# fan-ziqi/robot_lab

Hardware: AMD Instinct MI355X
Metric: env-steps/sec (whole node) at 4096 envs/GPU, A1 Velocity-Rough (higher is better)
Workload: dtype f32; 1 GPU; RobotLab-Isaac-Velocity-Rough-Unitree-A1-v0, 4096 envs/GPU, random actions U(-1,1), seed 42+rank; envs_per_gpu=4096, parallelism=env-shard x1, step_kernel=specialised (spec_id 1), envs_per_wavefront=4

## Files before the change

robot_lab_amd/csrc/env_spec.h:

```cpp
#pragma once
#include <string.h>

#include "env_tables.h"

namespace rl {

struct RewSpec {
  int kind;
  float weight;
  float p[4];
  uint32_t joint_mask;
  uint64_t body_mask;
  int n_idx;
  int idx_a[16], idx_b[16];
};
struct ObsSpec {
  int kind;
  float scale, clip_lo, clip_hi, noise_lo, noise_hi;
  int has_noise, offset;
};
struct NoSpec {
  static constexpr bool ON = false;
  static constexpr int ID = 0;
  static constexpr uint32_t SLOT_VALID = ~0u;
// ... 15 lines not shown
    if (kd == 37  || kd == 38 )
      for (int i = 0; i < SP::REW[t].n_idx; ++i) m |= 1ull << SP::REW[t].idx_a[i];
  }
  return m;
}
template <class SP>
constexpr int spec_axis_kind(int j) {
  if constexpr (SP::ON) return SP::AXIS_KIND[j];
  else return 3;
}
template <class LT>
inline int table_axis_kind(const LT& L, int j) {
  int kind = 3;
  for (int i = 0; i < 3; ++i) {
    const float a = L.axis[j][i], b = L.axis[j][(i + 1) % 3], c = L.axis[j][(i + 2) % 3];
    if ((a == 1.0f || a == -1.0f) && b == 0.0f && c == 0.0f) kind = i;
  }
  return kind;
}
template <class SP>
constexpr uint32_t spec_slot_valid() {
#ifdef RL_SLOT_VALID_ALL
  return ~0u;
#else
  return SP::SLOT_VALID;
#endif
}
template <class SP>
constexpr bool spec_slot_any(int s, int spl, int g_lo, int g_hi) {
  for (int g = g_lo; g <= g_hi; ++g)
    if ((spec_slot_valid<SP>() >> (g * spl + s)) & 1u) return true;
  return false;
}
constexpr bool spec_kind_supported(int kd) {
  return kd >= 0 && kd <= 38;
}

template <class SP>
inline bool spec_matches(const TablesT<TopoMax>& T) {
  auto same = [](float a, float b) { return memcmp(&a, &b, 4) == 0; };
  if (T.CL != SP::TP::CL || T.NW != SP::TP::NW || (T.merged != 0) != (SP::TP::M0 != 0) || (T.rotpad != 0) != (SP::TP::NW == 0 && SP::TP::PAD) || T.D != SP::D ||
      T.n_bodies != SP::N_BODIES)
    return false;
  if (T.n_rewards != SP::N_REW || T.cur_lin || T.cur_ang) return false;
  if (T.slot_valid != SP::SLOT_VALID) return false;
  for (int j = 0; j < SP::TP::CL; ++j)
    for (int k = 0; k < NLANE; ++k)
      if (SP::AXIS_KIND[j] != 3 && table_axis_kind(T.lane[k], j) != SP::AXIS_KIND[j]) return false;
  int owned = 0;
  for (int k = 0; k < NLANE; ++k)
    for (int j = 0; j < T.CL + T.NW; ++j) {
      const int jid = T.lane[k].joint_own[j] ? T.lane[k].joint_id[j] : -1;
      if (jid < 0) continue;
      ++owned;
      if (jid >= SP::D || SP::JOINT_K[jid] != k || SP::JOINT_J[jid] != j) return false;
    }
  if (owned != SP::D) return false;
  for (int t = 0; t < SP::N_REW; ++t) {
    const RewTab& R = T.rew[t];
    const RewSpec& Q = SP::REW[t];
    if (R.kind != Q.kind || !same(R.weight, Q.weight) || R.joint_mask != Q.joint_mask || R.body_mask != Q.body_mask || R.n_idx != Q.n_idx) return false;
    for (int i = 0; i < 4; ++i)
      if (!same(R.p[i], Q.p[i])) return false;
    const int nidx = R.kind == 20  ? 4 : R.n_idx;
    for (int i = 0; i < nidx; ++i)
      if (T.idx_pool_a[R.idx_off + i] != Q.idx_a[i] || T.idx_pool_b[R.idx_off + i] != Q.idx_b[i]) return false;
// ... 19 lines not shown
```

robot_lab_amd/csrc/env_step.h:

```cpp
#pragma once
#include <type_traits>

#include "env_spec.h"
#include "env_tables.h"

#if !defined(RL_NO_PK) && !defined(RL_PK)
#define RL_PK 1
#endif
#if defined(RL_PHASE_MARKS) && defined(__HIP_DEVICE_COMPILE__)
#define RL_PHASE(id, name) asm volatile("; PHASE " name)
#elif defined(RL_PHASE_CLOCK) && defined(__HIP_DEVICE_COMPILE__)
#define RL_PHASE(id, name) this->phase_stamp(id)
#define RL_PHASE_START() (this->ph_t0 = 0, this->ph_cur = 0)
#define RL_PHASE_CLOCK_ON 1
#else
#define RL_PHASE(id, name) ((void)0)
#endif
#ifndef RL_PHASE_START
#define RL_PHASE_START() ((void)0)
#endif
constexpr int RL_PHASE_ROW0 = 24;
constexpr int RL_PHASE_SLOTS = 32;

namespace rl {

template <int N>
struct SymIdx {
  static constexpr int size = N * (N + 1) / 2;
  static constexpr int at(int i, int j) { return i <= j ? i * N - i * (i - 1) / 2 + (j - i) : j * N - j * (j - 1) / 2 + (i - j); }
};

template <int I, int N, class F>
RL_FN void static_for(F&& f) {
  if constexpr (I < N) {
    f(std::integral_constant<int, I>{});
    static_for<I + 1, N>(f);
  }
}
template <int I, class F>
RL_FN void static_for_down(F&& f) {
  if constexpr (I >= 0) {
    f(std::integral_constant<int, I>{});
    static_for_down<I - 1>(f);
  }
}

RL_FN float comp(V3 v, int i) { return i == 0 ? v.x : i == 1 ? v.y : v.z; }
RL_FN V3 unit(int i) { return {i == 0 ? 1.f : 0.f, i == 1 ? 1.f : 0.f, i == 2 ? 1.f : 0.f}; }
RL_FN V3 ld3(const float* p) { return {p[0], p[1], p[2]}; }

struct Uni {
  float dt, inv_dt, gravity, contact_k, contact_c, inv_phi_ref, contact_ct, contact_vdep, contact_vstick, limit_k, limit_c, force_threshold;
  float inv_hscale, x0, y0;
  int is_plane, nx, ny;
  double x0d, y0d, inv_hd;
// ... 641 lines not shown
    k = ctx.k();
    sub = ctx.sub();
    li = k * SUB + sub;
    Np = S.Npad;
#pragma unroll
    for (int i = 0; i < MAXOWN; ++i) {
      if constexpr (SUB == 8) own[i] = -1;
      else own[i] = SUB == 1 ? i : (SUB == 2 ? L.own_slot2[sub & 1][i < LaneTabT<TP>::MAXOWN2 ? i : 0] : L.own_slot[sub & 3][i < LaneTabT<TP>::MAXOWN ? i : 0]);
    }
    if constexpr (SUB == 8) {
      int n = 0;
#pragma unroll
      for (int sl = 0; sl < NBS; ++sl) {
        const bool mine = (L.slot_body[sl] >= 0 || (sl == 0 && L.base_body_local >= 0)) && (L.slot_grp[sl] & 7) == sub;
#pragma unroll
        for (int i = 0; i < MAXOWN; ++i) own[i] = (mine && n == i) ? sl : own[i];
        n += mine ? 1 : 0;
      }
    }
    tim.set_own(own); hist_n.set_own(own); cf.set_own(own); fric.set_own(own);
    if constexpr (STATE_BUF) {
      lt_b = Ctx::state_buf(ctx.uniform_ptr(S.lane_state + (size_t)ctx.tile() * ((size_t)LY.NF_LANE * ROW)), (uint32_t)LY.NF_LANE * ROW * (uint32_t)sizeof(float));
      et_b = Ctx::state_buf(ctx.uniform_ptr(S.env_state + (size_t)ctx.tile() * ((size_t)LY.NF_ENV * EPT)), (uint32_t)LY.NF_ENV * (uint32_t)EPT * (uint32_t)sizeof(float));
      lt_off = (uint32_t)sizeof(float) * (uint32_t)(ctx.env_in_tile() * NLANE + k);
      et_off = (uint32_t)sizeof(float) * (uint32_t)ctx.env_in_tile();
    } else {
      lt = S.lane_state + (size_t)ctx.tile() * ((size_t)LY.NF_LANE * ROW) + (uint32_t)(ctx.env_in_tile() * NLANE + k);
      et = S.env_state + (size_t)ctx.tile() * ((size_t)LY.NF_ENV * EPT) + (uint32_t)ctx.env_in_tile();
    }
  }
#ifdef RL_PHASE_CLOCK_ON
  long long ph_t0 = 0;
  int ph_cur = 0;
  __device__ __forceinline__ void phase_stamp(int id) {
    __builtin_amdgcn_s_waitcnt(0);
    const long long t = (long long)__builtin_readcyclecounter();
    if (ctx.lane == 0 && ph_t0 != 0) {
      float* row = S.rew_terms + (size_t)RL_PHASE_ROW0 * (size_t)S.Npad + (size_t)ctx.tile() * RL_PHASE_SLOTS;
      row[ph_cur] += (float)(t - ph_t0);
    }
    ph_cur = id;
    __builtin_amdgcn_s_waitcnt(0);
    ph_t0 = (long long)__builtin_readcyclecounter();
  }
#endif
  RL_FN auto LF(int f) const {
    if constexpr (STATE_BUF) {
      const uint32_t o = (uint32_t)f * ROW * (uint32_t)sizeof(float);
      return __builtin_constant_p(f) ? BufRef{lt_b, lt_off, o} : BufRef{lt_b, lt_off + o, 0u};
    } else return PtrRef{lt + (uint32_t)f * ROW};
  }
  RL_FN auto EF(int f) const {
    if constexpr (STATE_BUF) {
      const uint32_t o = (uint32_t)f * (uint32_t)EPT * (uint32_t)sizeof(float);
      return __builtin_constant_p(f) ? BufRef{et_b, et_off, o} : BufRef{et_b, et_off + o, 0u};
    } else return PtrRef{et + (uint32_t)f * (uint32_t)EPT};
  }
  static constexpr bool M0 = TP::M0 != 0;
  static constexpr int G0 = M0 ? 1 : 0;
  RL_FN int grp_of(int it) const { return G0 + sub + SUB * it; }
  static constexpr bool slot_live(int it, int s) {
    const int lo = G0 + SUB * it, hi = lo + SUB - 1 < CL ? lo + SUB - 1 : CL;
    return spec_slot_any<SP>(s, SPL, lo, hi);
  }
  RL_FN bool owns_group(int g) const { return SUB == 1 || (g < G0 ? sub == 0 : ((g - G0) % SUB) == sub); }
  RL_FN bool on_base(int g, int s) const { return M0 && ((L.sph_base_mask >> (g * SPL + s)) & 1u) != 0u; }
  RL_FN static SV pick_sv(bool c, const SV& a, const SV& b) {
    return SV{{c ? a.a.x : b.a.x, c ? a.a.y : b.a.y, c ? a.a.z : b.a.z}, {c ? a.l.x : b.l.x, c ? a.l.y : b.l.y, c ? a.l.z : b.l.z}};
  }
  RL_FN uint32_t base_bits() const { return M0 ? L.sph_base_mask : ((1u << SPL) - 1u); }
  RL_FN bool owns_slot(int s) const { return owns_group(L.slot_grp[s]); }

  RL_FN void load() {
    pos = {EF(LY.EF_ROOT + 0), EF(LY.EF_ROOT + 1), EF(LY.EF_ROOT + 2)};
    quat = {EF(LY.EF_ROOT + 3), EF(LY.EF_ROOT + 4), EF(LY.EF_ROOT + 5), EF(LY.EF_ROOT + 6)};
    vlin = {EF(LY.EF_ROOT + 7), EF(LY.EF_ROOT + 8), EF(LY.EF_ROOT + 9)};
    vang = {EF(LY.EF_ROOT + 10), EF(LY.EF_ROOT + 11), EF(LY.EF_ROOT + 12)};
    extF = {EF(LY.EF_WRENCH + 0), EF(LY.EF_WRENCH + 1), EF(LY.EF_WRENCH + 2)};
    extT = {EF(LY.EF_WRENCH + 3), EF(LY.EF_WRENCH + 4), EF(LY.EF_WRENCH + 5)};
    base_com = {EF(LY.EF_BASE_COM + 0), EF(LY.EF_BASE_COM + 1), EF(LY.EF_BASE_COM + 2)};
    if (NW > 0) wr_com = {EF(LY.EF_WR_COM + 0), EF(LY.EF_WR_COM + 1), EF(LY.EF_WR_COM + 2)};
    else wr_com = base_com;
#pragma unroll
    for (int j = 0; j < CL; ++j) {
      q[j] = LF(LY.LF_Q + j);
      qd[j] = LF(LY.LF_QD + j);
      kp[j] = LF(LY.LF_KP + j);
      kd[j] = LF(LY.LF_KD + j);
      act[j] = LF(LY.LF_ACT + j);
    }
#pragma unroll
    for (int i = 0; i < NW; ++i) {
      q[CL + i] = EF(LY.EF_TQ + i);
      qd[CL + i] = EF(LY.EF_TQD + i);
      kp[CL + i] = EF(LY.EF_TKP + i);
      kd[CL + i] = EF(LY.EF_TKD + i);
      act[CL + i] = EF(LY.EF_TACT + i);
    }
#pragma unroll
    for (int j = 0; j < JX; ++j) {
      tau_app[j] = 0.f;
      qacc[j] = 0.f;
    }
    if (M0) {
#pragma unroll
// ... 1505 lines not shown
```

robot_lab_amd/csrc/env_terms.h:

```cpp
#pragma once
#include "env_spec.h"
#include "env_step.h"

namespace rl {

enum RewKind {
  REW_TRACK_LIN_VEL_XY_EXP = 0, REW_TRACK_ANG_VEL_Z_EXP, REW_LIN_VEL_Z_L2, REW_ANG_VEL_XY_L2, REW_JOINT_TORQUES_L2,
  REW_JOINT_ACC_L2, REW_JOINT_POS_LIMITS, REW_JOINT_POWER, REW_STAND_STILL, REW_JOINT_POS_PENALTY, REW_JOINT_MIRROR,
  REW_ACTION_RATE_L2, REW_UNDESIRED_CONTACTS, REW_CONTACT_FORCES, REW_FEET_CONTACT_WITHOUT_CMD, REW_FEET_HEIGHT_BODY,
  REW_UPWARD, REW_FEET_AIR_TIME, REW_FEET_AIR_TIME_VARIANCE, REW_FEET_SLIDE, REW_FEET_GAIT, REW_FLAT_ORIENTATION_L2,
  REW_IS_TERMINATED, REW_JOINT_DEVIATION_L1, REW_JOINT_VEL_L2, REW_FEET_CONTACT, REW_FEET_STUMBLE, REW_FEET_HEIGHT,
  REW_TRACK_LIN_VEL_XY_YAW_FRAME_EXP, REW_TRACK_ANG_VEL_Z_WORLD_EXP, REW_FEET_AIR_TIME_POSITIVE_BIPED,
  REW_HANDSTAND_FEET_HEIGHT_EXP, REW_HANDSTAND_FEET_ON_AIR, REW_HANDSTAND_FEET_AIR_TIME, REW_HANDSTAND_ORIENTATION_L2, REW_BASE_HEIGHT_L2, REW_WHEEL_VEL_PENALTY,
  REW_FEET_DISTANCE_Y_EXP, REW_FEET_DISTANCE_XY_EXP, REW_ACTION_MIRROR, REW_ACTION_SYNC
};
enum ObsKind {
  OBS_BASE_LIN_VEL = 0, OBS_BASE_ANG_VEL, OBS_PROJECTED_GRAVITY, OBS_VELOCITY_COMMANDS, OBS_JOINT_POS_REL,
  OBS_JOINT_VEL_REL, OBS_LAST_ACTION, OBS_HEIGHT_SCAN, OBS_JOINT_POS_REL_NO_WHEEL
};

enum { JS_TAU2 = 0, JS_ACC2, JS_QD2, JS_LIMIT, JS_POWER, JS_DEV1, JS_DEV2, JS_DA2, JS_Q, JS_ABSQD, JS_ROWS };
enum { BT_HMAX = 0, BT_CA, BT_CC, BT_LA, BT_LC, BT_FX, BT_FY, BT_FZ, BT_PX, BT_PY, BT_PZ, BT_VX, BT_VY, BT_VZ, BT_NF };
static_assert(JS_ROWS == REW_JS_ROWS && BT_NF == REW_BT_NF && BT_FX == REW_BT_NS, "reward tables: LDS sizing in env_tables.h");

// ... 309 lines not shown
  using Base::pos; using Base::quat; using Base::vlin; using Base::vang; using Base::q; using Base::qd; using Base::kp; using Base::kd;
  using Base::act; using Base::prev_act; using Base::tim; using Base::cf; using Base::hist_n; using Base::tau_app; using Base::qacc;
  using Base::extF; using Base::extT; using Base::base_com; using Base::wr_com;

  V3 cmd;
  float heading_target, cmd_time_left, metric_xy, metric_yaw, push_left;
  static constexpr bool DEFER_LOG = SUB > 1;
  static constexpr int NACC_M = (MAX_T + LPE - 1) / LPE;
  float log_sum[NACC_M], log_mxy, log_myaw;
  bool is_heading, is_standing;
  int level, ttype;
  V3 origin;
  long long ep_len;
  M3 Rwb;
  V3 lin_b, ang_b, grav_b, lin_w;
  float yaw_c, yaw_s;

  RL_FN EnvProgram(Ctx& c, const KState& s) : Base(c, s) {}

  RL_FN void load_task() {
    cmd = {this->EF(LY.EF_CMD + CMD_VX), this->EF(LY.EF_CMD + CMD_VY), this->EF(LY.EF_CMD + CMD_WZ)};
    heading_target = this->EF(LY.EF_CMD + CMD_HEADING);
    cmd_time_left = this->EF(LY.EF_CMD + CMD_TIME_LEFT);
    metric_xy = this->EF(LY.EF_CMD + CMD_METRIC_XY);
    metric_yaw = this->EF(LY.EF_CMD + CMD_METRIC_YAW);
    push_left = this->EF(LY.EF_CMD + CMD_PUSH_LEFT);
    int f = S.flags[e];
    is_heading = f & 1;
    is_standing = (f >> 1) & 1;
    level = S.level[e];
    ttype = S.ttype[e];
    origin = {this->EF(LY.EF_ORIGIN + 0), this->EF(LY.EF_ORIGIN + 1), this->EF(LY.EF_ORIGIN + 2)};
    ep_len = S.ep_len[e];
  }
  RL_FN void store_task() {
    if (li != 0) return;
    this->EF(LY.EF_CMD + CMD_VX) = cmd.x; this->EF(LY.EF_CMD + CMD_VY) = cmd.y; this->EF(LY.EF_CMD + CMD_WZ) = cmd.z;
    this->EF(LY.EF_CMD + CMD_HEADING) = heading_target; this->EF(LY.EF_CMD + CMD_TIME_LEFT) = cmd_time_left;
    this->EF(LY.EF_CMD + CMD_METRIC_XY) = metric_xy; this->EF(LY.EF_CMD + CMD_METRIC_YAW) = metric_yaw; this->EF(LY.EF_CMD + CMD_PUSH_LEFT) = push_left;
    S.flags[e] = (is_heading ? 1 : 0) | (is_standing ? 2 : 0);
    S.level[e] = level;
    this->EF(LY.EF_ORIGIN + 0) = origin.x; this->EF(LY.EF_ORIGIN + 1) = origin.y; this->EF(LY.EF_ORIGIN + 2) = origin.z;
    S.ep_len[e] = ep_len;
    S.command_out[e * 3 + 0] = cmd.x; S.command_out[e * 3 + 1] = cmd.y; S.command_out[e * 3 + 2] = cmd.z;
  }

  RL_FN void derive() {
    Rwb = quat_to_mat(quat);
    V3 com_w = mul(Rwb, base_com);
    lin_w = vlin + cross(vang, com_w);
    lin_b = mulT(Rwb, lin_w);
    ang_b = mulT(Rwb, vang);
    grav_b = mulT(Rwb, V3{0.f, 0.f, -1.f});
    const float hn = frsqrt(fmaxf(Rwb.r0.x * Rwb.r0.x + Rwb.r1.x * Rwb.r1.x, 1e-30f));
    yaw_c = Rwb.r0.x * hn;
    yaw_s = Rwb.r1.x * hn;
  }

  RL_FN uint64_t uniform_u64(uint64_t v) const {
    return ((uint64_t)(uint32_t)ctx.uniform_i((int)(uint32_t)(v >> 32)) << 32) | (uint64_t)(uint32_t)ctx.uniform_i((int)(uint32_t)v);
  }
  RL_FN float U(uint32_t stream, uint32_t idx, float lo, float hi) const {
    return uniform_range(S.seed, (uint32_t)e, S.step_counter, stream, idx, lo, hi);
  }

  RL_FN void apply_command_draws(const float (&uw)[6]) {
// ... 750 lines not shown
      uniform01x4(S.seed, (uint32_t)e, S.step_counter, STREAM_NOISE, (noise_base >> 2) + (uint32_t)b, un);
#pragma unroll
      for (int c = 0; c < 4; ++c) {
        const int col = 4 * b + c;
        if (col >= dim) continue;
        const bool in_scan = col >= scan_off && col < scan_off + scan_n;
        const int n = col < scan_off ? col : col - scan_n;
        const ObsColTab& dc = in_scan ? G.scan : G.col[in_scan ? 0 : n];
        stage[col] = clampf(stage[col] + fmaf(dc.noise_rng, un[c], dc.noise_lo), dc.clip_lo, dc.clip_hi) * dc.scale;
      }
    }
  }

  struct ScanAhead {
    ScanPatches sp;
    float cy, sy;
    V3 scan_p;
  };
  RL_FN void scan_ahead(bool chain_fresh, ScanAhead& A) {
    derive();
    scanner_pose(A.cy, A.sy, A.scan_p, chain_fresh);
    scan_fetch(A.cy, A.sy, A.scan_p, A.sp);
  }
  RL_FN void observations(bool chain_fresh) {
    ScanAhead A;
    scan_ahead(chain_fresh, A);
    observations(A);
  }
  RL_FN void observations_spec(const ScanAhead& A) {
    derive();
    Ctx& cx = ctx;
    const int my_li = li, my_sub = sub;
    const uint32_t wheel = T.wheel_joint_mask;
    static_for<0, 2>([&](auto gc) __attribute__((always_inline)) {
      constexpr int g = decltype(gc)::value;
      float* stage = cx.obs_stage(g);
      const bool corrupt = SP::OBS_CORRUPT[g] != 0 && cx.uniform_i(this->T.obs[g].corrupt) != 0;
      static_for<0, SP::N_OBS[g]>([&](auto tc) __attribute__((always_inline)) {
        constexpr int tm = decltype(tc)::value;
        constexpr ObsSpec O = SP::OBS[g][tm];
        auto fin = [&](float v) __attribute__((always_inline)) { return corrupt ? v : clampf(v, O.clip_lo, O.clip_hi) * O.scale; };
        if constexpr (O.kind == OBS_BASE_LIN_VEL || O.kind == OBS_BASE_ANG_VEL || O.kind == OBS_PROJECTED_GRAVITY || O.kind == OBS_VELOCITY_COMMANDS) {
          const V3 v = O.kind == OBS_BASE_LIN_VEL ? this->lin_b : (O.kind == OBS_BASE_ANG_VEL ? this->ang_b : (O.kind == OBS_PROJECTED_GRAVITY ? this->grav_b : this->cmd));
          if (my_li == 0) {
            stage[O.offset + 0] = fin(v.x);
            stage[O.offset + 1] = fin(v.y);
            stage[O.offset + 2] = fin(v.z);
          }
        } else if constexpr (O.kind == OBS_HEIGHT_SCAN) {
#ifndef RL_ABL_NO_SCAN
          this->write_scan(stage, O.offset, cx.uniform_i(this->T.scan_nx * this->T.scan_ny), corrupt, O.scale, O.clip_lo, O.clip_hi, A.cy, A.sy, A.scan_p, A.sp);
#endif
        } else {
          if (my_sub == 0) {
            static_for<0, JX>([&](auto jc) __attribute__((always_inline)) {
              constexpr int j = decltype(jc)::value;
              const int jid = (!TP::PAD || this->L.joint_own[j]) ? this->L.joint_id[j] : -1;
              if (jid >= 0) {
                const float qr = this->q[j] - this->L.q0[j];
                float v;
                if constexpr (O.kind == OBS_JOINT_POS_REL) v = qr;
                else if constexpr (O.kind == OBS_JOINT_VEL_REL) v = this->qd[j] - this->L.qd0[j];
                else if constexpr (O.kind == OBS_LAST_ACTION) v = this->act[j];
                else v = ((wheel >> (jid & 31)) & 1u) ? 0.f : qr;
                stage[O.offset + jid] = fin(v);
              }
            });
          }
        }
      });
      if (corrupt) {
        const auto& G = this->T.obs[g];
        this->noise_pass(G, stage, g == 0 ? 0u : 1024u, cx.uniform_i(G.dim), cx.uniform_i(G.scan_off), cx.uniform_i(G.scan_n));
      }
      if constexpr (g == 0) RL_PHASE(21, "obs.policy_done");
    });
    RL_PHASE(22, "obs.flush");
    ctx.flush_obs(S.obs_policy, T.policy_dim, 0);
    ctx.flush_obs(S.obs_critic, T.critic_dim, 1);
  }
  RL_FN void observations(const ScanAhead& A) {
#ifndef RL_SPEC_OBS_OFF
    if constexpr (SP::ON && SUB > 1 && NW == 0) {
      observations_spec(A);
      return;
    }
#endif
    derive();
    const ScanPatches& sp = A.sp;
    const float cy = A.cy, sy = A.sy;
    const V3 scan_p = A.scan_p;
    float* F = ctx.feat_stage();
    const int D = ctx.uniform_i(T.D);
    if (li == 0) {
      F[FEAT_LIN + 0] = lin_b.x; F[FEAT_LIN + 1] = lin_b.y; F[FEAT_LIN + 2] = lin_b.z;
      F[FEAT_ANG + 0] = ang_b.x; F[FEAT_ANG + 1] = ang_b.y; F[FEAT_ANG + 2] = ang_b.z;
      F[FEAT_GRAV + 0] = grav_b.x; F[FEAT_GRAV + 1] = grav_b.y; F[FEAT_GRAV + 2] = grav_b.z;
      F[FEAT_CMD + 0] = cmd.x; F[FEAT_CMD + 1] = cmd.y; F[FEAT_CMD + 2] = cmd.z;
    }
    if (sub == 0) {
      const uint32_t wheel = T.wheel_joint_mask;
#pragma unroll
      for (int j = 0; j < JX; ++j) {
        const int jid = (!TP::PAD || L.joint_own[j]) ? L.joint_id[j] : -1;
        if (jid < 0) continue;
        const float qr = q[j] - L.q0[j];
        F[FEAT_JOINT + jid] = qr;
        F[FEAT_JOINT + D + jid] = qd[j] - L.qd0[j];
        F[FEAT_JOINT + 2 * D + jid] = act[j];
        F[FEAT_JOINT + 3 * D + jid] = ((wheel >> (jid & 31)) & 1u) ? 0.f : qr;
      }
    }
// ... 16 lines not shown
  RL_FN void collect_cmd_levels(bool done) {
    if (!(T.cur_lin || T.cur_ang) || !done || e >= S.N || S.step_counter % (uint32_t)T.max_episode_length != 0u) return;
    for (int t = li; t < T.n_rewards; t += LPE) {
      const float v = S.ep_sums[(size_t)t * Np + e];
      if (T.cur_lin && t == T.cur_lin_term) { ctx.atomic_add(S.cmd_levels + CL_SUM_LIN, v); ctx.atomic_add(S.cmd_levels + CL_CNT_LIN, 1.f); }
      if (T.cur_ang && t == T.cur_ang_term) { ctx.atomic_add(S.cmd_levels + CL_SUM_ANG, v); ctx.atomic_add(S.cmd_levels + CL_CNT_ANG, 1.f); }
    }
  }
  RL_FN void write_dbg_views(float live) {
    if (S.dbg_torque == nullptr) return;
    if (sub == 0)
#pragma unroll
      for (int j = 0; j < JX; ++j) {
        if (TP::PAD && !L.joint_own[j]) continue;
        S.dbg_torque[(size_t)e * T.D + L.joint_id[j]] = live * tau_app[j];
        S.dbg_acc[(size_t)e * T.D + L.joint_id[j]] = live * qacc[j];
      }
#pragma unroll
    for (int s = 0; s < NBS; ++s) {
      int b = L.slot_body[s];
      if (b >= 0 && (s != 0 || L.owns_base_body) && this->owns_slot(s)) {
        float* o = S.dbg_cforce + ((size_t)e * T.n_bodies + b) * 3;
        const F4 fs = cf.ld(s);
        o[0] = live * fs.x; o[1] = live * fs.y; o[2] = live * fs.z;
      }
    }
  }
  RL_FN bool out_of_bounds() const {
    if (!T.term_oob || T.is_plane) return false;
    const float mw = (float)T.num_rows * T.tile_size + 2.f * T.border, mh = (float)T.num_cols * T.tile_size + 2.f * T.border;
    return fabsf(pos.x) > 0.5f * mw - T.oob_buffer || fabsf(pos.y) > 0.5f * mh - T.oob_buffer;
  }

  RL_FN void step() { step_front<false>(); }
  RL_FN void step_head() { step_front<true>(); }
  RL_FN void step_tail() {
    this->load();
    load_task();
    derive();
    const bool terminated = S.terminated[e] != 0, time_out = S.time_out[e] != 0;
    const bool t_oob = out_of_bounds();
    const bool t_timeout = T.term_time_out && ep_len >= (long long)T.max_episode_length;
    step_back<true>(terminated, time_out, t_timeout, t_oob, terminated);
  }

  template <bool HEAD>
  RL_FN void step_front() {
    constexpr size_t LOG_SLOT_WORDS = (size_t)LOG_PARTS * LOG_SIZE;
    const int log_tl = ctx.tile(), log_wl = ctx.env_in_tile() * LPE + li;
    float* log_pv = S.log + (size_t)((S.step_counter - 1u) & (uint32_t)(LOG_RING - 1)) * LOG_SLOT_WORDS;
    const float* log_pp = S.log + (size_t)((S.step_counter - 2u) & (uint32_t)(LOG_RING - 1)) * LOG_SLOT_WORDS;
    float log_fresh = 0.f, log_word = 0.f;
    if (log_tl < LOG_PARTS) {
      for (int p = 0; p < LOG_PARTS; ++p) log_fresh += log_pv[p * LOG_SIZE + LOG_FRESH];
      log_word = log_pp[log_tl * LOG_SIZE + log_wl];
    }
    float a_in[JX];
    {
      const float* arow = S.action_in + (size_t)(e < S.N ? e : 0) * T.D;
#pragma unroll
      for (int j = 0; j < JX; ++j) {
        const int jid = L.joint_id[j];
        a_in[j] = arow[TP::PAD && jid < 0 ? 0 : jid];
      }
    }
    RL_PHASE_START();
    RL_PHASE(0, "load");
    this->load();
    load_task();
    rl_pin(a_in);
    if (log_tl < LOG_PARTS) {
      float* nx = S.log + (size_t)((S.step_counter + 1u) & (uint32_t)(LOG_RING - 1)) * LOG_SLOT_WORDS;
      const bool inherit = log_fresh == 0.f;
      if (inherit && log_wl != LOG_FRESH) log_pv[log_tl * LOG_SIZE + log_wl] = log_word;
      nx[log_tl * LOG_SIZE + log_wl] = 0.f;
      for (int p = log_tl + S.Npad / (64 / LPE); p < LOG_PARTS; p += S.Npad / (64 / LPE)) {
        if (inherit && log_wl != LOG_FRESH) log_pv[p * LOG_SIZE + log_wl] = log_pp[p * LOG_SIZE + log_wl];
        nx[p * LOG_SIZE + log_wl] = 0.f;
      }
    }
    RL_PHASE(1, "action");
    float q_tgt[JX], qd_tgt[JX];
#pragma unroll
    for (int j = 0; j < JX; ++j) {
      prev_act[j] = act[j];
      const float a = (e < S.N && (!TP::PAD || L.joint_id[j] >= 0)) ? a_in[j] : 0.f;
      act[j] = a;
      float pr = clampf(a * L.a_scale[j] + L.a_off[j], L.a_lo[j], L.a_hi[j]);
      q_tgt[j] = L.action_is_vel[j] ? 0.f : pr;
      qd_tgt[j] = L.action_is_vel[j] ? pr : 0.f;
    }
#ifdef RL_ABL_SUBSTEPS
    if constexpr (Base::ABA) {
      this->substeps_aba(q_tgt, qd_tgt, RL_ABL_SUBSTEPS);
    } else
#endif
    if constexpr (Base::ABA) {
      this->substeps_aba(q_tgt, qd_tgt, T.decimation);
    } else {
      this->self_load();
      for (int s = 0; s < T.decimation; ++s) this->substep_aba_trunk(q_tgt, qd_tgt);
    }
// ... 112 lines not shown
    RL_PHASE(20, "observations");
#ifndef RL_ABL_NO_OBS
#ifdef RL_SCAN_EARLY
    observations(scanA);
#else
    observations(!TAIL && !ctx.any(terminated || time_out));
#endif
#endif
#ifndef RL_ABL_NO_LOG
    if constexpr (DEFER_LOG) {
      if (sums_folded && e < S.N) {
        float* slot = log_slot();
        int n_rew;
        if constexpr (SP::ON) n_rew = SP::N_REW;
        else n_rew = T.n_rewards;
#pragma unroll
        for (int i = 0; i < NACC_M; ++i) {
          const int t = li + LPE * i;
          if (t < n_rew) ctx.atomic_add(slot + LOG_EP_SUM0 + t, log_sum[i]);
        }
        if (li == 0) {
          ctx.atomic_add(slot + LOG_RESET_COUNT, 1.0f);
          ctx.atomic_add(slot + LOG_FRESH, 1.0f);
          ctx.atomic_add(slot + LOG_METRIC_XY, log_mxy);
          ctx.atomic_add(slot + LOG_METRIC_YAW, log_myaw);
          if (t_timeout) ctx.atomic_add(slot + LOG_TERM_TIMEOUT, 1.f);
          if (t_oob) ctx.atomic_add(slot + LOG_TERM_OOB, 1.f);
          if (t_illegal) ctx.atomic_add(slot + LOG_TERM_ILLEGAL, 1.f);
        }
      }
    }
#endif
    RL_PHASE(24, "end");
  }

  RL_FN void reset_entry() {
    if (S.mode == KMODE_STEP_TAIL) {
      step_tail();
      return;
    }
    this->load();
    load_task();
#pragma unroll
    for (int j = 0; j < JX; ++j) prev_act[j] = act[j];
    if (S.reset_mask == nullptr || S.reset_mask[e]) reset_env(false);
    observations(false);
    this->store();
    store_task();
  }
};

}
```

robot_lab_amd/csrc/rl_env_kernels.h:

```cpp
#pragma once
#include <hip/hip_runtime.h>

#include <algorithm>
#include <cmath>
#include <cstdlib>
#include <mutex>
#include <string>

#define RL_FN __host__ __device__ __forceinline__
#include "env_aos.h"
#include "env_terms.h"

namespace {

using namespace rl;

template <int CTRL>
__device__ inline float dpp(float v) {
  return __int_as_float(__builtin_amdgcn_update_dpp(0, __float_as_int(v), CTRL, 0xF, 0xF, false));
}
template <int CTRL>
__device__ inline float dpp_move(float v) {
  return __int_as_float(__builtin_amdgcn_update_dpp(0, __float_as_int(v), CTRL, 0xF, 0xF, true));
}
// ... 197 lines not shown
  P.rtdim = rew_tab_words(D, n_bodies, rew_ext_mask);
  P.rsdim = rew_stage_words(n_rewards);
  int region = P.s0w + P.s1w + EPT * P.fdim;
  if (region < EPT * P.rtdim) P.s1w += EPT * P.rtdim - region, region = EPT * P.rtdim;
  if (SUB > 1 && region < EPT * RESET_RAND_WORDS) P.s1w += EPT * RESET_RAND_WORDS - region, region = EPT * RESET_RAND_WORDS;
  P.lb0 = LS::WORDS * 64;
  P.lbrec0 = P.lb0 + LbLayout<TP>::CHAINW * LIMBS;
  P.envs = P.lb0 + LbLayout<TP>::WORDS * LIMBS;
  P.tail = P.envs + EPT * LbLayout<TP>::ENV_WORDS;
  const bool alias = TP::NW == 0 && STASH_WORDS > 0 && EPT * P.rsdim + region <= STASH_WORDS;
  const bool alias_lb = TP::NW > 0 && EPT * P.rsdim + region <= LB_FREE;
  P.rstage = alias ? LS::CT * 64 : (alias_lb ? P.lbrec0 : P.tail);
  P.stage0 = P.rstage + EPT * P.rsdim;
  P.stage1 = P.stage0 + P.s0w;
  P.fstage = P.stage1 + P.s1w;
  P.words = (alias || alias_lb) ? P.tail : P.tail + EPT * P.rsdim + region;
  P.words = (P.words + 3) & ~3;
  return P;
}

extern __shared__ float4 smem4[];

#ifndef RL_LB
#define RL_LB(w) 256
#endif
template <class TP, int RESET, int SUB, int WGW, class SP = NoSpec>
__global__ __launch_bounds__(RL_LB(WGW)) void env_kernel(KState S, const void* __restrict__ Tgv, uint32_t wave_words) {
  using Ctx = WaveCtx<SUB>;
  using Tables = TablesT<TP>;
  const Tables* __restrict__ Tg = static_cast<const Tables*>(Tgv);
  float* smem = reinterpret_cast<float*>(smem4);
  Tables* Tl = reinterpret_cast<Tables*>(smem);
  const int lane = threadIdx.x & 63, wv = threadIdx.x >> 6;
  S.step_counter += *S.step_base;
  {
    const float4* src = reinterpret_cast<const float4*>(Tg);
    float4* dst = reinterpret_cast<float4*>(Tl);
    constexpr int TPB = 64 * WGW;
    constexpr int NIT = ((int)(sizeof(Tables) / 16) + TPB - 1) / TPB;
    const int n4 = (int)(S.table_bytes >> 4);
    float4 tmp[NIT];
#pragma unroll
    for (int it = 0; it < NIT; ++it) {
      const int i = (int)threadIdx.x + TPB * it;
      tmp[it] = src[i < n4 ? i : n4 - 1];
    }
#pragma unroll
    for (int it = 0; it < NIT; ++it) {
      const int i = (int)threadIdx.x + TPB * it;
      if (i < n4) dst[i] = tmp[it];
    }
  }
  if (WGW > 1) __syncthreads();
  else Ctx::wave_sync();
  const int TAB_F = (int)(S.table_bytes >> 2);
  const LdsPlan P = lds_plan<TP, SUB>(Tl->policy_dim, Tl->critic_dim, direct_group(*Tl, 0), direct_group(*Tl, 1), Tl->D, Tl->n_bodies, Tl->rew_ext_mask, Tl->n_rewards);
  Ctx ctx;
  ctx.T = Tl;
  ctx.Tg = Tgv;
  ctx.dim[0] = Tl->policy_dim;
  ctx.dim[1] = Tl->critic_dim;
  ctx.lscratch = smem + TAB_F + (WGW > 1 ? wv * wave_words : 0u);
  ctx.wtile = (int)blockIdx.x * WGW + wv;
  if (WGW > 1 && ctx.wtile >= S.Npad / Ctx::EPT) return;
  ctx.lbchain = ctx.lscratch + P.lb0 + (lane / SUB) * LbLayout<TP>::CHAINW;
  ctx.lbrec = ctx.lscratch + P.lbrec0 + (lane / SUB) * LbLayout<TP>::RECW;
  ctx.lbrec_stride = LbLayout<TP>::RECW;
  ctx.envs = ctx.lscratch + P.envs + (lane / Ctx::LPE) * LbLayout<TP>::ENV_WORDS;
  ctx.fdim = P.fdim;
  ctx.rtdim = P.rtdim;
  ctx.rsdim = P.rsdim;
  ctx.rstage = ctx.lscratch + P.rstage;
  ctx.stage[0] = ctx.lscratch + P.stage0;
  ctx.stage[1] = ctx.lscratch + P.stage1;
  ctx.fstage = ctx.lscratch + P.fstage;
  ctx.lane = lane;
  EnvProgram<Ctx, TP, SP> prog(ctx, S);
  if (RESET == 1)
    prog.reset_entry();
  else if (RESET == 2)
    prog.step_head();
  else
    prog.step();
}


struct LaunchCfg {
  int device = 0, n_cu = 256;
  int wg_waves = 4;
  bool wg_force = false;
};

template <class TP, int SUB, int WGW, class SP = NoSpec>
hipError_t launch_w(const LaunchCfg& cfg, const KState& S, const void* T, size_t lds1, hipStream_t st) {
  const int tiles = S.Npad / (16 / SUB);
  dim3 grid((tiles + WGW - 1) / WGW), block(64 * WGW);
  const uint32_t wave_words = (uint32_t)((lds1 - S.table_bytes) >> 2);
  const size_t lds = S.table_bytes + (size_t)WGW * (lds1 - S.table_bytes);
  constexpr bool HEAD = SUB == 4 && WGW == 1 && !SP::ON, RESET = WGW == 1 && !SP::ON;
  if (lds > 64 * 1024) {
    static size_t configured[64] = {};
    static std::mutex mu;
    std::lock_guard<std::mutex> lock(mu);
    size_t& have = configured[cfg.device & 63];
    if (lds > have) {
      hipError_t e = hipFuncSetAttribute(reinterpret_cast<const void*>(&env_kernel<TP, 0, SUB, WGW, SP>), hipFuncAttributeMaxDynamicSharedMemorySize, (int)lds);
      if (e != hipSuccess) return e;
      if constexpr (RESET) {
        e = hipFuncSetAttribute(reinterpret_cast<const void*>(&env_kernel<TP, 1, SUB, WGW>), hipFuncAttributeMaxDynamicSharedMemorySize, (int)lds);
        if (e != hipSuccess) return e;
      }
      if constexpr (HEAD) {
        e = hipFuncSetAttribute(reinterpret_cast<const void*>(&env_kernel<TP, 2, SUB, WGW>), hipFuncAttributeMaxDynamicSharedMemorySize, (int)lds);
        if (e != hipSuccess) return e;
// ... 50 lines not shown
```

Baseline: 131.2 million env-steps/s.

## Prefetch per-env state into registers while staging tables into LDS

Global loads of per-env and per-lane state (root pose, joint fields, command, flags, owned timer/friction rows, actions, log words) are issued in the kernel prologue alongside the table copy into LDS, then placed into program state from registers. This hides global-load latency behind the table staging and barrier instead of loading serially after setup. It raises register pressure through the large Pre struct, which may reduce occupancy or cause spills. It also adds phase-clock instrumentation and an optional early obs-flush ordering behind macros.

```diff
diff --git a/robot_lab_amd/csrc/env_spec.h b/robot_lab_amd/csrc/env_spec.h
--- a/robot_lab_amd/csrc/env_spec.h
+++ b/robot_lab_amd/csrc/env_spec.h
@@ -71,6 +71,22 @@
     if ((spec_slot_valid<SP>() >> (g * spl + s)) & 1u) return true;
   return false;
 }
+template <class SP>
+constexpr int spec_joint_at(int k, int j) {
+  if constexpr (SP::ON) {
+    for (int jid = 0; jid < SP::D; ++jid)
+      if (SP::JOINT_K[jid] == k && SP::JOINT_J[jid] == j) return jid;
+  }
+  return -1;
+}
+template <class SP, class TP>
+constexpr bool spec_joints_dense() {
+  if (!SP::ON || TP::NW != 0 || TP::PAD) return false;
+  for (int k = 0; k < NLANE; ++k)
+    for (int j = 0; j < TP::JX; ++j)
+      if (spec_joint_at<SP>(k, j) < 0) return false;
+  return true;
+}
 constexpr bool spec_kind_supported(int kd) {
   return kd >= 0 && kd <= 38;
 }
diff --git a/robot_lab_amd/csrc/env_step.h b/robot_lab_amd/csrc/env_step.h
--- a/robot_lab_amd/csrc/env_step.h
+++ b/robot_lab_amd/csrc/env_step.h
@@ -11,7 +11,8 @@
 #define RL_PHASE(id, name) asm volatile("; PHASE " name)
 #elif defined(RL_PHASE_CLOCK) && defined(__HIP_DEVICE_COMPILE__)
 #define RL_PHASE(id, name) this->phase_stamp(id)
-#define RL_PHASE_START() (this->ph_t0 = 0, this->ph_cur = 0)
+#define RL_PHASE_START() ((void)0)
+#define RL_PHASE_END() this->phase_stamp(RL_PHASE_SLOTS - 1)
 #define RL_PHASE_CLOCK_ON 1
 #else
 #define RL_PHASE(id, name) ((void)0)
@@ -19,8 +20,12 @@
 #ifndef RL_PHASE_START
 #define RL_PHASE_START() ((void)0)
 #endif
+#ifndef RL_PHASE_END
+#define RL_PHASE_END() ((void)0)
+#endif
 constexpr int RL_PHASE_ROW0 = 24;
-constexpr int RL_PHASE_SLOTS = 32;
+constexpr int RL_PHASE_SLOTS = 40;
+constexpr int RL_PHASE_HEAD_STAGE = 32, RL_PHASE_HEAD_PLAN = 33;
 
 namespace rl {
 
@@ -728,6 +733,15 @@
 #ifdef RL_PHASE_CLOCK_ON
   long long ph_t0 = 0;
   int ph_cur = 0;
+  __device__ __forceinline__ void phase_head(long long t_entry, long long t_staged) {
+    __builtin_amdgcn_s_waitcnt(0);
+    if (ctx.lane == 0) {
+      float* row = S.rew_terms + (size_t)RL_PHASE_ROW0 * (size_t)S.Npad + (size_t)ctx.tile() * RL_PHASE_SLOTS;
+      row[RL_PHASE_HEAD_STAGE] += (float)(t_staged - t_entry);
+    }
+    ph_cur = RL_PHASE_HEAD_PLAN;
+    ph_t0 = t_staged;
+  }
   __device__ __forceinline__ void phase_stamp(int id) {
     __builtin_amdgcn_s_waitcnt(0);
     const long long t = (long long)__builtin_readcyclecounter();
@@ -767,6 +781,137 @@
   RL_FN uint32_t base_bits() const { return M0 ? L.sph_base_mask : ((1u << SPL) - 1u); }
   RL_FN bool owns_slot(int s) const { return owns_group(L.slot_grp[s]); }
 
+#ifdef RL_NO_HEAD_PREFETCH
+  static constexpr bool HEAD_PREFETCH = false;
+#else
+  static constexpr bool HEAD_PREFETCH = !STATE_BUF;
+#endif
+  static constexpr bool PRE_OWN = NW == 0;
+  static constexpr bool PRE_ACT = spec_joints_dense<SP, TP>();
+  struct Pre {
+    float ef[LY.NF_ENV], lf[LY.NF_LANE];
+    int own[MAXOWN];
+    float own_w[MAXOWN][7];
+    int flags, level, ttype;
+    long long ep_len;
+    float a_in[JX];
+    float log_fresh[LOG_PARTS], log_word;
+  };
+  RL_FN static void prefetch(const KState& S, int tile, int env_in_tile, int kk, Pre& P) {
+    const int e_ = tile * EPT + env_in_tile;
+    const float* lt_ = S.lane_state + (size_t)tile * ((size_t)LY.NF_LANE * ROW) + (uint32_t)(env_in_tile * NLANE + kk);
+    const float* et_ = S.env_state + (size_t)tile * ((size_t)LY.NF_ENV * EPT) + (uint32_t)env_in_tile;
+    auto ef = [&](int f0, int n) __attribute__((always_inline)) {
+#pragma unroll
+      for (int i = 0; i < n; ++i) P.ef[f0 + i] = et_[(uint32_t)(f0 + i) * (uint32_t)EPT];
+    };
+    auto lf = [&](int f0, int n) __attribute__((always_inline)) {
+#pragma unroll
+      for (int i = 0; i < n; ++i) P.lf[f0 + i] = lt_[(uint32_t)(f0 + i) * ROW];
+    };
+    lf(LY.LF_Q, 5 * CL);
+    if constexpr (PRE_ACT) {
+      const float* arow = S.action_in + (size_t)(e_ < S.N ? e_ : 0) * SP::D;
+#pragma unroll
+      for (int j = 0; j < JX; ++j) {
+        const int jid = kk == 0 ? spec_joint_at<SP>(0, j) : (kk == 1 ? spec_joint_at<SP>(1, j) : (kk == 2 ? spec_joint_at<SP>(2, j) : spec_joint_at<SP>(3, j)));
+        P.a_in[j] = arow[jid];
+      }
+    }
+    ef(LY.EF_ROOT, 19);
+    ef(LY.EF_BASE_COM, 3);
+    if constexpr (NW > 0) {
+      ef(LY.EF_WR_COM, 3);
+      ef(LY.EF_TQ, 5 * NW);
+    }
+    ef(LY.EF_CMD, CMD_NFIELD + 3);
+    P.flags = S.flags[e_];
+    P.level = S.level[e_];
+    P.ttype = S.ttype[e_];
+    P.ep_len = S.ep_len[e_];
+    if constexpr (PRE_OWN && M0) lf(LY.LF_FRICTION, 3);
+  }
+  RL_FN static void prefetch_own(const TablesT<TP>& Tg, int kk, int sub_, Pre& P) {
+    if constexpr (PRE_OWN) {
+      const LaneTabT<TP>& Lg = Tg.lane[kk];
+#pragma unroll
+      for (int i = 0; i < MAXOWN; ++i)
+        P.own[i] = SUB == 1 ? i : (SUB == 2 ? Lg.own_slot2[sub_ & 1][i < LaneTabT<TP>::MAXOWN2 ? i : 0] : Lg.own_slot[sub_ & 3][i < LaneTabT<TP>::MAXOWN ? i : 0]);
+    }
+  }
+  RL_FN static void prefetch_own_rows(const KState& S, int tile, int env_in_tile, int kk, Pre& P) {
+    if constexpr (PRE_OWN) {
+      const float* lt_ = S.lane_state + (size_t)tile * ((size_t)LY.NF_LANE * ROW) + (uint32_t)(env_in_tile * NLANE + kk);
+#pragma unroll
+      for (int i = 0; i < MAXOWN; ++i) {
+        const uint32_t s = (uint32_t)(P.own[i] < 0 ? 0 : P.own[i]);
+#pragma unroll
+        for (int t = 0; t < 4; ++t) P.own_w[i][t] = lt_[((uint32_t)LY.LF_TIMERS + s * 4u + (uint32_t)t) * ROW];
+#pragma unroll
+        for (int t = 0; t < 3; ++t) P.own_w[i][4 + t] = lt_[((uint32_t)LY.LF_FRICTION + s * 3u + (uint32_t)t) * ROW];
+      }
+    }
+  }
+  RL_FN static void prefetch_log(const KState& S, int tile, int env_in_tile, int li_, int lane0, Pre& P) {
+    if (tile < LOG_PARTS) {
+      constexpr size_t LOG_SLOT_WORDS = (size_t)LOG_PARTS * LOG_SIZE;
+      const float* log_pv = S.log + (size_t)((S.step_counter - 1u) & (uint32_t)(LOG_RING - 1)) * LOG_SLOT_WORDS;
+      const float* log_pp = S.log + (size_t)((S.step_counter - 2u) & (uint32_t)(LOG_RING - 1)) * LOG_SLOT_WORDS;
+#pragma unroll
+      for (int p = 0; p < LOG_PARTS; ++p) P.log_fresh[p] = log_pv[p * LOG_SIZE + LOG_FRESH + lane0];
+      P.log_word = log_pp[tile * LOG_SIZE + env_in_tile * LPE + li_];
+    }
+  }
+  RL_FN void load_placed(const Pre& P) {
+    pos = {P.ef[LY.EF_ROOT + 0], P.ef[LY.EF_ROOT + 1], P.ef[LY.EF_ROOT + 2]};
+    quat = {P.ef[LY.EF_ROOT + 3], P.ef[LY.EF_ROOT + 4], P.ef[LY.EF_ROOT + 5], P.ef[LY.EF_ROOT + 6]};
+    vlin = {P.ef[LY.EF_ROOT + 7], P.ef[LY.EF_ROOT + 8], P.ef[LY.EF_ROOT + 9]};
+    vang = {P.ef[LY.EF_ROOT + 10], P.ef[LY.EF_ROOT + 11], P.ef[LY.EF_ROOT + 12]};
+    extF = {P.ef[LY.EF_WRENCH + 0], P.ef[LY.EF_WRENCH + 1], P.ef[LY.EF_WRENCH + 2]};
+    extT = {P.ef[LY.EF_WRENCH + 3], P.ef[LY.EF_WRENCH + 4], P.ef[LY.EF_WRENCH + 5]};
+    base_com = {P.ef[LY.EF_BASE_COM + 0], P.ef[LY.EF_BASE_COM + 1], P.ef[LY.EF_BASE_COM + 2]};
+    if constexpr (NW > 0) wr_com = {P.ef[LY.EF_WR_COM + 0], P.ef[LY.EF_WR_COM + 1], P.ef[LY.EF_WR_COM + 2]};
+    else wr_com = base_com;
+#pragma unroll
+    for (int j = 0; j < CL; ++j) {
+      q[j] = P.lf[LY.LF_Q + j];
+      qd[j] = P.lf[LY.LF_QD + j];
+      kp[j] = P.lf[LY.LF_KP + j];
+      kd[j] = P.lf[LY.LF_KD + j];
+      act[j] = P.lf[LY.LF_ACT + j];
+    }
+#pragma unroll
+    for (int i = 0; i < NW; ++i) {
+      q[CL + i] = P.ef[LY.EF_TQ + i];
+      qd[CL + i] = P.ef[LY.EF_TQD + i];
+      kp[CL + i] = P.ef[LY.EF_TKP + i];
+      kd[CL + i] = P.ef[LY.EF_TKD + i];
+      act[CL + i] = P.ef[LY.EF_TACT + i];
+    }
+#pragma unroll
+    for (int j = 0; j < JX; ++j) {
+      tau_app[j] = 0.f;
+      qacc[j] = 0.f;
+    }
+    if (M0) {
+#pragma unroll
+      for (int t = 0; t < 3; ++t) fric0[t] = P.lf[LY.LF_FRICTION + t];
+    }
+#pragma unroll
+    for (int i = 0; i < MAXOWN; ++i) {
+      const int s = own[i];
+      if (s < 0) continue;
+      if constexpr (PRE_OWN) {
+        tim.st(s, F4{P.own_w[i][0], P.own_w[i][1], P.own_w[i][2], P.own_w[i][3]});
+        fric.st(s, F4{P.own_w[i][4], P.own_w[i][5], P.own_w[i][6], 0.f});
+      } else {
+        tim.st(s, F4{LF(LY.LF_TIMERS + s * 4 + 0), LF(LY.LF_TIMERS + s * 4 + 1), LF(LY.LF_TIMERS + s * 4 + 2), LF(LY.LF_TIMERS + s * 4 + 3)});
+        fric.st(s, F4{LF(LY.LF_FRICTION + s * 3 + 0), LF(LY.LF_FRICTION + s * 3 + 1), LF(LY.LF_FRICTION + s * 3 + 2), 0.f});
+      }
+      cf.st(s, F4{0.f, 0.f, 0.f, 0.f});
+      hist_n.st(s, F4{0.f, 0.f, 0.f, 0.f});
+    }
+  }
   RL_FN void load() {
     pos = {EF(LY.EF_ROOT + 0), EF(LY.EF_ROOT + 1), EF(LY.EF_ROOT + 2)};
     quat = {EF(LY.EF_ROOT + 3), EF(LY.EF_ROOT + 4), EF(LY.EF_ROOT + 5), EF(LY.EF_ROOT + 6)};
diff --git a/robot_lab_amd/csrc/env_terms.h b/robot_lab_amd/csrc/env_terms.h
--- a/robot_lab_amd/csrc/env_terms.h
+++ b/robot_lab_amd/csrc/env_terms.h
@@ -365,6 +365,20 @@
     ttype = S.ttype[e];
     origin = {this->EF(LY.EF_ORIGIN + 0), this->EF(LY.EF_ORIGIN + 1), this->EF(LY.EF_ORIGIN + 2)};
     ep_len = S.ep_len[e];
+  }
+  RL_FN void load_task_placed(const typename Base::Pre& P) {
+    cmd = {P.ef[LY.EF_CMD + CMD_VX], P.ef[LY.EF_CMD + CMD_VY], P.ef[LY.EF_CMD + CMD_WZ]};
+    heading_target = P.ef[LY.EF_CMD + CMD_HEADING];
+    cmd_time_left = P.ef[LY.EF_CMD + CMD_TIME_LEFT];
+    metric_xy = P.ef[LY.EF_CMD + CMD_METRIC_XY];
+    metric_yaw = P.ef[LY.EF_CMD + CMD_METRIC_YAW];
+    push_left = P.ef[LY.EF_CMD + CMD_PUSH_LEFT];
+    is_heading = P.flags & 1;
+    is_standing = (P.flags >> 1) & 1;
+    level = P.level;
+    ttype = P.ttype;
+    origin = {P.ef[LY.EF_ORIGIN + 0], P.ef[LY.EF_ORIGIN + 1], P.ef[LY.EF_ORIGIN + 2]};
+    ep_len = P.ep_len;
   }
   RL_FN void store_task() {
     if (li != 0) return;
@@ -1181,8 +1195,13 @@
     Ctx& cx = ctx;
     const int my_li = li, my_sub = sub;
     const uint32_t wheel = T.wheel_joint_mask;
+#ifdef RL_OBS_FLUSH_EARLY
+    constexpr bool FLUSH_EARLY = true;
+#else
+    constexpr bool FLUSH_EARLY = false;
+#endif
     static_for<0, 2>([&](auto gc) __attribute__((always_inline)) {
-      constexpr int g = decltype(gc)::value;
+      constexpr int g = FLUSH_EARLY ? 1 - decltype(gc)::value : decltype(gc)::value;
       float* stage = cx.obs_stage(g);
       const bool corrupt = SP::OBS_CORRUPT[g] != 0 && cx.uniform_i(this->T.obs[g].corrupt) != 0;
       static_for<0, SP::N_OBS[g]>([&](auto tc) __attribute__((always_inline)) {
@@ -1222,11 +1241,21 @@
         const auto& G = this->T.obs[g];
         this->noise_pass(G, stage, g == 0 ? 0u : 1024u, cx.uniform_i(G.dim), cx.uniform_i(G.scan_off), cx.uniform_i(G.scan_n));
       }
-      if constexpr (g == 0) RL_PHASE(21, "obs.policy_done");
+      if constexpr (FLUSH_EARLY) {
+        if constexpr (g == 1) {
+          cx.flush_obs(this->S.obs_critic, this->T.critic_dim, 1);
+          RL_PHASE(21, "obs.policy_done");
+        } else {
+          RL_PHASE(22, "obs.flush");
+          cx.flush_obs(this->S.obs_policy, this->T.policy_dim, 0);
+        }
+      } else if constexpr (g == 0) RL_PHASE(21, "obs.policy_done");
     });
-    RL_PHASE(22, "obs.flush");
-    ctx.flush_obs(S.obs_policy, T.policy_dim, 0);
-    ctx.flush_obs(S.obs_critic, T.critic_dim, 1);
+    if constexpr (!FLUSH_EARLY) {
+      RL_PHASE(22, "obs.flush");
+      ctx.flush_obs(S.obs_policy, T.policy_dim, 0);
+      ctx.flush_obs(S.obs_critic, T.critic_dim, 1);
+    }
   }
   RL_FN void observations(const ScanAhead& A) {
 #ifndef RL_SPEC_OBS_OFF
@@ -1309,8 +1338,20 @@
     return fabsf(pos.x) > 0.5f * mw - T.oob_buffer || fabsf(pos.y) > 0.5f * mh - T.oob_buffer;
   }
 
-  RL_FN void step() { step_front<false>(); }
-  RL_FN void step_head() { step_front<true>(); }
+  using Pre = typename Base::Pre;
+  static constexpr bool HEAD_PREFETCH = Base::HEAD_PREFETCH;
+  RL_FN void step() {
+    if constexpr (HEAD_PREFETCH) {
+      Pre P;
+      Base::prefetch_own(T, k, sub, P);
+      Base::prefetch(S, ctx.tile(), ctx.env_in_tile(), k, P);
+      Base::prefetch_own_rows(S, ctx.tile(), ctx.env_in_tile(), k, P);
+      Base::prefetch_log(S, ctx.tile(), ctx.env_in_tile(), li, 0, P);
+      step_front<false>(P);
+    } else step_front<false>(Pre{});
+  }
+  RL_FN void step(const Pre& P) { step_front<false>(P); }
+  RL_FN void step_head() { step_front<true>(Pre{}); }
   RL_FN void step_tail() {
     this->load();
     load_task();
@@ -1322,18 +1363,24 @@
   }
 
   template <bool HEAD>
-  RL_FN void step_front() {
+  RL_FN void step_front(const Pre& P) {
+    constexpr bool PLACED = HEAD_PREFETCH && !HEAD;
     constexpr size_t LOG_SLOT_WORDS = (size_t)LOG_PARTS * LOG_SIZE;
     const int log_tl = ctx.tile(), log_wl = ctx.env_in_tile() * LPE + li;
     float* log_pv = S.log + (size_t)((S.step_counter - 1u) & (uint32_t)(LOG_RING - 1)) * LOG_SLOT_WORDS;
     const float* log_pp = S.log + (size_t)((S.step_counter - 2u) & (uint32_t)(LOG_RING - 1)) * LOG_SLOT_WORDS;
     float log_fresh = 0.f, log_word = 0.f;
-    if (log_tl < LOG_PARTS) {
-      for (int p = 0; p < LOG_PARTS; ++p) log_fresh += log_pv[p * LOG_SIZE + LOG_FRESH];
-      log_word = log_pp[log_tl * LOG_SIZE + log_wl];
+    if constexpr (!PLACED) {
+      if (log_tl < LOG_PARTS) {
+        for (int p = 0; p < LOG_PARTS; ++p) log_fresh += log_pv[p * LOG_SIZE + LOG_FRESH];
+        log_word = log_pp[log_tl * LOG_SIZE + log_wl];
+      }
     }
     float a_in[JX];
-    {
+    if constexpr (PLACED && Base::PRE_ACT) {
+#pragma unroll
+      for (int j = 0; j < JX; ++j) a_in[j] = P.a_in[j];
+    } else {
       const float* arow = S.action_in + (size_t)(e < S.N ? e : 0) * T.D;
 #pragma unroll
       for (int j = 0; j < JX; ++j) {
@@ -1343,8 +1390,18 @@
     }
     RL_PHASE_START();
     RL_PHASE(0, "load");
-    this->load();
-    load_task();
+    if constexpr (PLACED) {
+      this->load_placed(P);
+      load_task_placed(P);
+      if (log_tl < LOG_PARTS) {
+#pragma unroll
+        for (int p = 0; p < LOG_PARTS; ++p) log_fresh += P.log_fresh[p];
+        log_word = P.log_word;
+      }
+    } else {
+      this->load();
+      load_task();
+    }
     rl_pin(a_in);
     if (log_tl < LOG_PARTS) {
       float* nx = S.log + (size_t)((S.step_counter + 1u) & (uint32_t)(LOG_RING - 1)) * LOG_SLOT_WORDS;
@@ -1523,6 +1580,7 @@
     }
 #endif
     RL_PHASE(24, "end");
+    RL_PHASE_END();
   }
 
   RL_FN void reset_entry() {
diff --git a/robot_lab_amd/csrc/rl_env_kernels.h b/robot_lab_amd/csrc/rl_env_kernels.h
--- a/robot_lab_amd/csrc/rl_env_kernels.h
+++ b/robot_lab_amd/csrc/rl_env_kernels.h
@@ -253,7 +253,15 @@
   float* smem = reinterpret_cast<float*>(smem4);
   Tables* Tl = reinterpret_cast<Tables*>(smem);
   const int lane = threadIdx.x & 63, wv = threadIdx.x >> 6;
+#ifdef RL_PHASE_CLOCK_ON
+  const long long ph_entry = (long long)__builtin_readcyclecounter();
+#endif
   S.step_counter += *S.step_base;
+  using Prog = EnvProgram<Ctx, TP, SP>;
+  constexpr bool PREFETCH = RESET == 0 && Prog::HEAD_PREFETCH;
+  typename Prog::Pre pre;
+  const int pre_tile = (int)blockIdx.x * WGW + wv < S.Npad / Ctx::EPT ? (int)blockIdx.x * WGW + wv : S.Npad / Ctx::EPT - 1;
+  if constexpr (PREFETCH) Prog::prefetch_own(*Tg, (lane / SUB) & 3, lane & (SUB - 1), pre);
   {
     const float4* src = reinterpret_cast<const float4*>(Tg);
     float4* dst = reinterpret_cast<float4*>(Tl);
@@ -266,14 +274,31 @@
       const int i = (int)threadIdx.x + TPB * it;
       tmp[it] = src[i < n4 ? i : n4 - 1];
     }
+    if constexpr (PREFETCH) {
+      __builtin_amdgcn_sched_barrier(0);
+      Prog::prefetch(S, pre_tile, lane / Ctx::LPE, (lane / SUB) & 3, pre);
+      __builtin_amdgcn_sched_barrier(0);
+      Prog::prefetch_own_rows(S, pre_tile, lane / Ctx::LPE, (lane / SUB) & 3, pre);
+#pragma unroll
+      for (int it = 0; it < NIT; ++it) { rl_pin(tmp[it].x); rl_pin(tmp[it].y); rl_pin(tmp[it].z); rl_pin(tmp[it].w); }
+    }
 #pragma unroll
     for (int it = 0; it < NIT; ++it) {
       const int i = (int)threadIdx.x + TPB * it;
       if (i < n4) dst[i] = tmp[it];
     }
   }
+  if constexpr (PREFETCH) {
+    int lane0 = 0;
+    rl_pin(lane0);
+    Prog::prefetch_log(S, pre_tile, lane / Ctx::LPE, lane & (Ctx::LPE - 1), lane0, pre);
+  }
   if (WGW > 1) __syncthreads();
   else Ctx::wave_sync();
+#ifdef RL_PHASE_CLOCK_ON
+  __builtin_amdgcn_s_waitcnt(0);
+  const long long ph_staged = (long long)__builtin_readcyclecounter();
+#endif
   const int TAB_F = (int)(S.table_bytes >> 2);
   const LdsPlan P = lds_plan<TP, SUB>(Tl->policy_dim, Tl->critic_dim, direct_group(*Tl, 0), direct_group(*Tl, 1), Tl->D, Tl->n_bodies, Tl->rew_ext_mask, Tl->n_rewards);
   Ctx ctx;
@@ -296,11 +321,16 @@
   ctx.stage[1] = ctx.lscratch + P.stage1;
   ctx.fstage = ctx.lscratch + P.fstage;
   ctx.lane = lane;
-  EnvProgram<Ctx, TP, SP> prog(ctx, S);
+  Prog prog(ctx, S);
+#ifdef RL_PHASE_CLOCK_ON
+  prog.phase_head(ph_entry, ph_staged);
+#endif
   if (RESET == 1)
     prog.reset_entry();
   else if (RESET == 2)
     prog.step_head();
+  else if constexpr (PREFETCH)
+    prog.step(pre);
   else
     prog.step();
 }
```

New measurement: 133.0 million env-steps/s (median of 6 runs). 1.4% higher.
